# jdfxzzy/DPMN

Measured on AMD Instinct MI355X. Metric: SR images/sec (16x64->32x128, bs=48 per GPU, fp32 forward), higher is better.
Workload: dtype f32; 1 GPU; cfg1: TATT PSN + 3+3 PGRM (embed 96, windows 2/4/8) + CMM, forward-only; per_gpu_batch=48, global_batch=48, ranks=1, batches_in_flight=2, parallelism=dp1 (independent batch shards, no forward collective)

## Files before the change

dpmn_amd/csrc/gemm.hip:

```cpp
#include "gemm_body.h"

namespace {

constexpr int WS_BM = 32, WS_BN = 96;

template <int EPI>
__device__ __forceinline__ void epilogue_fast(f32x4 (&acc)[3][1], int m0, int n0, int ldy, float* y, const float4 (&bias4)[3],
                                              const float* res1, const float* res2, float* red, int bn_cols, int n_block0) {
  const int lane = threadIdx.x & 63;
  const int lm = lane & 15, lq = lane >> 4;
  const size_t off = (size_t)(m0 + lm) * ldy + n0 + lq * 4;
  float4 r1[3], r2[3];
  if (EPI == 3 || EPI == 5) {
#pragma unroll
    for (int nt = 0; nt < 3; ++nt) {
      r1[nt] = *reinterpret_cast<const float4*>(res1 + off + nt * 16);
      if (EPI == 3) r2[nt] = *reinterpret_cast<const float4*>(res2 + off + nt * 16);
    }
  }
#pragma unroll
  for (int nt = 0; nt < 3; ++nt) {
    const float4 b4 = bias4[nt];
    float v[4] = {acc[nt][0][0] + b4.x, acc[nt][0][1] + b4.y, acc[nt][0][2] + b4.z, acc[nt][0][3] + b4.w};
    if (EPI == 2) {
// ... 770 lines not shown
      for (int nt = 0; nt < NT; ++nt) {
        f32x4 c4;
#pragma unroll
        for (int r = 0; r < 4; ++r) {
          float c = cs[nt][r];
          c += xshfl<1>(c); c += xshfl<2>(c); c += xshfl<4>(c); c += xshfl<8>(c);
          c4[r] = c;
        }
        if (lr == 0) *reinterpret_cast<f32x4*>(e.colsum + (size_t)(tile / SUB) * N + n_blk + 16 * nt + 4 * kq) = c4;
      }
    }
  }
}


template <int C, int CG, bool SAVE>
__global__ __launch_bounds__(256, 2) void k_sk_mlp_in(const float* __restrict__ cat, const float* __restrict__ sel, int rows_per_image,
                                                      const float* __restrict__ w_head, const float* __restrict__ b_head,
                                                      const float* __restrict__ feats, const float* __restrict__ shortcut, float* __restrict__ x1,
                                                      const float* __restrict__ ln_w, const float* __restrict__ ln_b, float eps,
                                                      const float* __restrict__ w_fc1, const float* __restrict__ b_fc1, float* __restrict__ y,
                                                      int M, int N, float* __restrict__ v_out, float* __restrict__ n2_out, float p_row,
                                                      unsigned long long seed_row) {
  constexpr int KC = C / 16, KV = C / 4, LDW = C + PAD, BN = 96, NT = 6, G = C / CG, HC = CG / 16, LDH = CG + PAD;
  static_assert(C == 96 && G == 3, "built for dim 96, three window groups");
  extern __shared__ __attribute__((aligned(16))) float smem[];
  float* Ws = smem;
  float* pb = Ws + BN * LDW;
  float* Wh = pb + 3 * BN;
  float* scr = Wh;
  const int tid = threadIdx.x, wave = tid >> 6, lane = tid & 63, lr = lane & 15, kq = lane >> 4;
  const int n_blk = blockIdx.y * BN;
  const int tiles = M / 16;
  const int stride = gridDim.x * 4;
  int tile = blockIdx.x * 4 + wave;
  const bool write_x1 = blockIdx.y == 0;

  constexpr int WL = (BN * KV + 255) / 256;
  float4 wv[WL];
#pragma unroll
  for (int u = 0; u < WL; ++u) {
    const int i = min(tid + u * 256, BN * KV - 1);
    wv[u] = *reinterpret_cast<const float4*>(w_fc1 + (size_t)(n_blk + i / KV) * C + (i % KV) * 4);
  }
  f32x4 xr[G][HC];
  auto load_rows = [&](int t_) {
    const size_t m = (size_t)(t_ < tiles ? t_ : tiles - 1) * 16 + lr;
#pragma unroll
    for (int g = 0; g < G; ++g)
#pragma unroll
      for (int c = 0; c < HC; ++c) xr[g][c] = *reinterpret_cast<const f32x4*>(cat + m * C + g * CG + 16 * c + 4 * kq);
  };
  f32x4 r1[NT], r2[NT];
  auto load_res = [&](int t_) {
    const size_t ro = ((size_t)(t_ < tiles ? t_ : tiles - 1) * 16 + lr) * C + 4 * kq;
#pragma unroll
    for (int nt = 0; nt < NT; ++nt) {
      r1[nt] = *reinterpret_cast<const f32x4*>(feats + ro + 16 * nt);
      r2[nt] = *reinterpret_cast<const f32x4*>(shortcut + ro + 16 * nt);
    }
  };
  load_rows(tile);
  load_res(tile);
#pragma unroll
  for (int u = 0; u < WL; ++u) {
    const int i = tid + u * 256;
    if (i < BN * KV) {
      const int r = i / KV, c4 = (i % KV) * 4;
      float4 v = wv[u];
      if (!SAVE) {
        const float4 gm = *reinterpret_cast<const float4*>(ln_w + c4), bt = *reinterpret_cast<const float4*>(ln_b + c4);
        const float4 wb = make_float4(v.x * bt.x, v.y * bt.y, v.z * bt.z, v.w * bt.w);
        v = make_float4(v.x * gm.x, v.y * gm.y, v.z * gm.z, v.w * gm.w);
        scr[r * KV + c4 / 4] = (wb.x + wb.y) + (wb.z + wb.w);
      }
      *reinterpret_cast<float4*>(Ws + r * LDW + c4) = v;
    }
  }
  __syncthreads();
  if (tid < BN) {
    float bb = b_fc1 ? b_fc1[n_blk + tid] : 0.f, cw = 0.f;
    if (!SAVE)
    for (int k = 0; k < KV; ++k) {
      const float4 v = *reinterpret_cast<const float4*>(Ws + tid * LDW + 4 * k);
      cw += (v.x + v.y) + (v.z + v.w);
      bb += scr[tid * KV + k];
    }
    pb[tid] = bb;
    pb[BN + tid] = cw;
    pb[2 * BN + tid] = b_head ? b_head[tid] : 0.f;
  }
  __syncthreads();
  for (int i = tid; i < C * (CG / 4); i += 256) {
    const int r = i / (CG / 4), c4 = (i % (CG / 4)) * 4;
    *reinterpret_cast<float4*>(Wh + r * LDH + c4) = *reinterpret_cast<const float4*>(w_head + (size_t)r * CG + c4);
  }
  __syncthreads();

  for (; tile < tiles; tile += stride) {
    const size_t m = (size_t)tile * 16 + lr;
    const size_t roff = m * C + 4 * kq;
    f32x4 xb[HC];
    {
      const size_t b = m / rows_per_image;
#pragma unroll
      for (int c = 0; c < HC; ++c) {
        xb[c] = (f32x4){0.f, 0.f, 0.f, 0.f};
#pragma unroll
        for (int g = 0; g < G; ++g) {
          const f32x4 a = *reinterpret_cast<const f32x4*>(sel + (b * G + g) * CG + 16 * c + 4 * kq);
// ... 14 lines not shown
    {
      const float* ha = Wh + lr * LDH + 4 * kq;
#pragma unroll
      for (int c = 0; c < HC; ++c) {
        f32x4 hf[NT];
#pragma unroll
        for (int nt = 0; nt < NT; ++nt) hf[nt] = *reinterpret_cast<const f32x4*>(ha + 16 * nt * LDH + 16 * c);
#pragma unroll
        for (int s4 = 0; s4 < 4; ++s4)
#pragma unroll
          for (int nt = 0; nt < NT; ++nt) x1r[nt] = mfma16(hf[nt][s4], xb[c][s4], x1r[nt]);
      }
    }
#pragma unroll
    for (int nt = 0; nt < NT; ++nt) {
      const f32x4 b4 = *reinterpret_cast<const f32x4*>(pb + 2 * BN + 16 * nt + 4 * kq);
      f32x4 v = x1r[nt] + b4;
      v += r1[nt];
      if (p_row > 0.f) v *= drop_scale(seed_row, (unsigned long long)(m / rows_per_image), p_row, 1.0f / (1.0f - p_row));
      v += r2[nt];
      x1r[nt] = v;
    }
    __builtin_amdgcn_sched_barrier(0);
    load_res(tile + stride);
    __builtin_amdgcn_sched_barrier(0);
    if (write_x1) {
#pragma unroll
      for (int nt = 0; nt < NT; ++nt) *reinterpret_cast<f32x4*>(x1 + roff + 16 * nt) = x1r[nt];
    }
    float mean, rstd;
    {
// ... 10 lines not shown
        q0 = fmaf(d0, d0, q0); q1 = fmaf(d1, d1, q1); q2 = fmaf(d2, d2, q2); q3 = fmaf(d3, d3, q3);
      }
      float q = (q0 + q1) + (q2 + q3);
      q += xshfl<16>(q); q += xshfl<32>(q);
      rstd = 1.0f / sqrtf(q * (1.0f / C) + eps);
    }
    if (SAVE) {
#pragma unroll
      for (int nt = 0; nt < NT; ++nt) {
        const f32x4 gm = *reinterpret_cast<const f32x4*>(ln_w + 16 * nt + 4 * kq), bt = *reinterpret_cast<const f32x4*>(ln_b + 16 * nt + 4 * kq);
#pragma unroll
        for (int r = 0; r < 4; ++r) x1r[nt][r] = (x1r[nt][r] - mean) * rstd * gm[r] + bt[r];
        if (write_x1) *reinterpret_cast<f32x4*>(n2_out + roff + 16 * nt) = x1r[nt];
      }
    }
    f32x4 acc[NT];
#pragma unroll
    for (int nt = 0; nt < NT; ++nt) acc[nt] = (f32x4){0.f, 0.f, 0.f, 0.f};
    const float* wa = Ws + lr * LDW + 4 * kq;
    f32x4 wf[2][NT];
#pragma unroll
    for (int nt = 0; nt < NT; ++nt) wf[0][nt] = *reinterpret_cast<const f32x4*>(wa + 16 * nt * LDW);
#pragma unroll
    for (int c = 0; c < KC; ++c) {
      if (c + 1 < KC) {
#pragma unroll
        for (int nt = 0; nt < NT; ++nt) wf[(c + 1) & 1][nt] = *reinterpret_cast<const f32x4*>(wa + 16 * nt * LDW + 16 * (c + 1));
      }
#pragma unroll
      for (int s4 = 0; s4 < 4; ++s4)
#pragma unroll
        for (int nt = 0; nt < NT; ++nt) acc[nt] = mfma16(wf[c & 1][nt][s4], x1r[c][s4], acc[nt]);
      __builtin_amdgcn_sched_barrier(0);
    }
    const float nm = -mean * rstd;
    const size_t yoff = m * N + n_blk + 4 * kq;
#pragma unroll
    for (int nt = 0; nt < NT; ++nt) {
      const f32x4 b4 = *reinterpret_cast<const f32x4*>(pb + 16 * nt + 4 * kq);
      const f32x4 cw = *reinterpret_cast<const f32x4*>(pb + BN + 16 * nt + 4 * kq);
      f32x4 v;
      if (SAVE) v = acc[nt] + b4;
      else {
#pragma unroll
        for (int r = 0; r < 4; ++r) v[r] = fmaf(acc[nt][r], rstd, fmaf(nm, cw[r], b4[r]));
      }
      *reinterpret_cast<f32x4*>(y + yoff + 16 * nt) = v;
    }
  }
}

template <int K, int PRO, int EPI>
int launch_rowreg(const float* x, int ldx, const float* w, float* y, int ldy, int M, int N, const ProArgs& p, const EpiArgs& e,
                  hipStream_t st) {
  const size_t smem = (size_t)(96 * (K + PAD) + 2 * 96 + (PRO == PRO_LN ? 96 * (K / 4) * 2 : 0)) * sizeof(float);
  static bool attr_set = false;
  if (!attr_set) {
    (void)hipFuncSetAttribute(reinterpret_cast<const void*>(&k_gemm_rowreg<K, PRO, EPI>), hipFuncAttributeMaxDynamicSharedMemorySize, (int)smem);
    attr_set = true;
  }
  const int tiles = M / (EPI == 4 ? 32 : 16), ny = N / 96;
  const bool x3 = (PRO == PRO_NONE || PRO == PRO_LN) && (K == 96 || K == 192) && g_dpmn_x3;
  const int per_cu = x3 ? (K <= 96 ? 2 : 1) : (smem <= 40 * 1024 ? 3 : (smem <= 80 * 1024 ? 2 : 1));
  int gx = 256 * per_cu / ny;
// ... 196 lines not shown
                       dpmn_stream_t stream) {
  return dpmn_sk_mlp_in_drop_f32(cat, attn_vec, w_head, b_head, feats, shortcut, x1, ln_w, ln_b, eps, w_fc1, b_fc1, y, v_out, n2_out, M,
                                 rows_per_image, C, groups, N, 0.f, 0ull, stream);
}

int dpmn_sk_mlp_in_drop_f32(const float* cat, const float* attn_vec, const float* w_head, const float* b_head, const float* feats,
                            const float* shortcut, float* x1, const float* ln_w, const float* ln_b, float eps, const float* w_fc1,
                            const float* b_fc1, float* y, float* v_out, float* n2_out, int M, int rows_per_image, int C, int groups, int N,
                            float p_row, unsigned long long seed_row, dpmn_stream_t stream) {
  DPMN_REQUIRE(p_row >= 0.f && p_row < 1.f, "sk_mlp_in: DropPath rate in [0, 1)");
  DPMN_REQUIRE(cat && attn_vec && w_head && feats && shortcut && x1 && ln_w && ln_b && w_fc1 && y, "sk_mlp_in: null pointer");
  DPMN_REQUIRE((v_out == nullptr) == (n2_out == nullptr), "sk_mlp_in: the two training outputs go together");
  DPMN_REQUIRE(C == 96 && groups == 3 && N % 96 == 0 && M % 16 == 0 && rows_per_image % 16 == 0 && M >= 1024,
               "sk_mlp_in: built for dim 96, three window groups, whole 16-token tiles (dpmn_sk_mlp_in_supported)");
  constexpr int Cc = 96, CG = 32;
  const size_t smem = (size_t)(96 * (Cc + PAD) + 3 * 96 + 96 * (CG + PAD)) * sizeof(float);
  static bool attr_set = false;
  if (!attr_set) {
    (void)hipFuncSetAttribute(reinterpret_cast<const void*>(&k_sk_mlp_in<Cc, CG, false>), hipFuncAttributeMaxDynamicSharedMemorySize, (int)smem);
    (void)hipFuncSetAttribute(reinterpret_cast<const void*>(&k_sk_mlp_in<Cc, CG, true>), hipFuncAttributeMaxDynamicSharedMemorySize, (int)smem);
    attr_set = true;
  }
  const int tiles = M / 16, ny = N / 96;
  int gx = 512 / ny;
  if (gx < 1) gx = 1;
  if (gx * 4 > tiles) gx = cdiv(tiles, 4);
  hipStream_t st = as_stream(stream);
  ProfScope prof(PT_GEMM_WSTAT_LN, st, 2.0 * M * ((double)N * Cc + (double)Cc * CG),
                 4.0 * ((double)M * Cc * 4 + (double)M * N + (double)N * Cc + (double)Cc * CG));
#define SKMLP_LAUNCH(SAVE_) hipLaunchKernelGGL((k_sk_mlp_in<Cc, CG, SAVE_>), dim3(gx, ny), dim3(256), smem, st, cat, attn_vec, rows_per_image, \
                                              w_head, b_head, feats, shortcut, x1, ln_w, ln_b, eps, w_fc1, b_fc1, y, M, N, v_out, n2_out, p_row, seed_row)
  if (g_dpmn_x3)
    dpmn_gemm::x3_launch_sk_mlp_in(cat, attn_vec, rows_per_image, w_head, b_head, feats, shortcut, x1, ln_w, ln_b, eps, w_fc1, b_fc1, y, M, N,
                                   v_out, n2_out, p_row, seed_row, gx, st);
  else if (v_out) SKMLP_LAUNCH(true);
  else SKMLP_LAUNCH(false);
#undef SKMLP_LAUNCH
  DPMN_CHECK_LAUNCH();
  return DPMN_OK;
}

int dpmn_sk_mlp_in_supported(int M, int rows_per_image, int C, int groups, int N) {
  return C == 96 && groups == 3 && N % 96 == 0 && M % 16 == 0 && rows_per_image % 16 == 0 && M >= 1024 && !g_dpmn_bf16;
}

int dpmn_pointwise_wgrad_f32(const float* dz, const float* g, float* dw, int B, int Ch, int L, dpmn_stream_t stream) {
  DPMN_REQUIRE(dz && g && dw && L % 32 == 0 && Ch % 4 == 0, "pointwise_wgrad: bad arguments");
  EpiArgs e{nullptr, nullptr, nullptr, nullptr, ACT_NONE, 0.f, 1};
  dim3 grid(cdiv(Ch, 64), cdiv(Ch, 96), 32);
  if (g_dpmn_x3) dpmn_gemm::x3_launch_kloop(dz, L, g, L, dw, Ch, Ch, Ch, B * L, e, L, (long)Ch * L, (long)Ch * L, grid, as_stream(stream));
  else hipLaunchKernelGGL(k_gemm_kloop, grid, dim3(256), 0, as_stream(stream), dz, L, g, L, dw, Ch, Ch, Ch, B * L, e, L,
                     (long)Ch * L, (long)Ch * L);
// ... 61 lines not shown
```

dpmn_amd/csrc/gemm_body.h:

```cpp
#pragma once
#include <cstdlib>
#include "common.h"

namespace dpmn_gemm {
struct EpiArgs {
  const float* bias;
  const float* res1;
  const float* res2;
  float* colsum;
  int act;
  float slope;
  int atomic;
  long zstride;
  float p_elem = 0.f, p_row = 0.f;
  unsigned long long seed_elem = 0ull, seed_row = 0ull;
  long row_len = 0;
};

struct ProArgs {
  const float* ln_w;
  const float* ln_b;
  float eps;
  const float* sel;
  int rows_per_image;
  int groups;
  const float* addv;
  const float* x2;
  int k1;
};

void x3_launch_kloop(const float* x, int ldx, const float* w, int ldw, float* y, int ldy, int M, int N, int K, const EpiArgs& e, int kb_len,
                     long x_bstride, long w_bstride, dim3 grid, hipStream_t st);
void x3_launch_kloop128(const float* x, const float* w, float* y, int M, int N, int L, int nchunks, int splits, long bstride, long zstride,
                        hipStream_t st);
void x3_launch_pw(const float* g, const float* w, const float* bias, float* z, int B, int Ch, int L, hipStream_t st);
int x3_launch_rowreg(int K, int pro, int epi, const float* x, int ldx, const float* w, float* y, int ldy, int M, int N, const ProArgs& p,
                     const EpiArgs& e, int gx, hipStream_t st);
void x3_launch_sk_mlp_in(const float* cat, const float* sel, int rows_per_image, const float* w_head, const float* b_head, const float* feats,
                         const float* shortcut, float* x1, const float* ln_w, const float* ln_b, float eps, const float* w_fc1, const float* b_fc1,
                         float* y, int M, int N, float* v_out, float* n2_out, float p_row, unsigned long long seed_row, int gx, hipStream_t st);
}

namespace {
using dpmn_gemm::EpiArgs;
using dpmn_gemm::ProArgs;
constexpr int PAD = 4;
enum { PRO_NONE = 0, PRO_LN = 1, PRO_SKSEL = 2, PRO_ADD = 3, PRO_CAT2 = 4 };

template <int NT, int MT, bool FULL = false>
__device__ __forceinline__ void epilogue(f32x4 (&acc)[NT][MT], int m0, int n0, int M, int N, int ldy, float* y,
                                         const EpiArgs& e, float* red , int bn_cols,
                                         int n_block0) {
  const int lane = threadIdx.x & 63;
  const int lm = lane & 15, lq = lane >> 4;
#pragma unroll
// ... 60 lines not shown
```

dpmn_amd/csrc/gemm_rowreg_x3.hip:

```cpp
#include <cstdlib>
#include "gemm_body.h"

namespace {
typedef unsigned u32x4 __attribute__((ext_vector_type(4)));

__device__ __forceinline__ void split_rows8(const f32x4& lo, const f32x4& hi, bf16x8& h, bf16x8& m, bf16x8& l) {
  u32x4 H, M_, L;
  unsigned a, b, c;
  x3_split2t(lo[0], lo[1], a, b, c); H[0] = a; M_[0] = b; L[0] = c;
  x3_split2t(lo[2], lo[3], a, b, c); H[1] = a; M_[1] = b; L[1] = c;
  x3_split2t(hi[0], hi[1], a, b, c); H[2] = a; M_[2] = b; L[2] = c;
  x3_split2t(hi[2], hi[3], a, b, c); H[3] = a; M_[3] = b; L[3] = c;
  h = __builtin_bit_cast(bf16x8, H); m = __builtin_bit_cast(bf16x8, M_); l = __builtin_bit_cast(bf16x8, L);
}

template <int K>
__device__ __forceinline__ void stage_w4(unsigned short* Wb, int r, int c4, const float4& v) {
  constexpr int LDB = K + 8, PL = 96 * LDB;
  uint2 h, m, l;
  x3_split4t(v, h, m, l);
  const int pos = (c4 & ~31) + 8 * ((c4 >> 2) & 3) + 4 * ((c4 >> 4) & 1);
  unsigned short* d = Wb + r * LDB + pos;
  *reinterpret_cast<uint2*>(d) = h;
  *reinterpret_cast<uint2*>(d + PL) = m;
  *reinterpret_cast<uint2*>(d + 2 * PL) = l;
}

template <int K, int NT>
__device__ __forceinline__ void mma_chunk(const unsigned short* Wb, int lr, int kq, int C2, const bf16x8& bh, const bf16x8& bm, const bf16x8& bl,
                                          f32x4 (&acc)[NT]) {
  constexpr int LDB = K + 8, PL = 96 * LDB;
  const unsigned short* wa = Wb + lr * LDB + 32 * C2 + 8 * kq;
  bf16x8 wh[NT], wm[NT], wl[NT];
#pragma unroll
  for (int nt = 0; nt < NT; ++nt) wl[nt] = *reinterpret_cast<const bf16x8*>(wa + 16 * nt * LDB + 2 * PL);
#pragma unroll
  for (int nt = 0; nt < NT; ++nt) wh[nt] = *reinterpret_cast<const bf16x8*>(wa + 16 * nt * LDB);
#pragma unroll
  for (int nt = 0; nt < NT; ++nt) wm[nt] = *reinterpret_cast<const bf16x8*>(wa + 16 * nt * LDB + PL);
#pragma unroll
  for (int nt = 0; nt < NT; ++nt) acc[nt] = mfma16_bf16(wl[nt], bh, acc[nt]);
#pragma unroll
  for (int nt = 0; nt < NT; ++nt) acc[nt] = mfma16_bf16(wh[nt], bl, acc[nt]);
#pragma unroll
  for (int nt = 0; nt < NT; ++nt) acc[nt] = mfma16_bf16(wm[nt], bm, acc[nt]);
#pragma unroll
// ... 132 lines not shown
#pragma unroll
      for (int nt = 0; nt < NT; ++nt) {
        f32x4 c4;
#pragma unroll
        for (int r = 0; r < 4; ++r) {
          float c = cs[nt][r];
          c += xshfl<1>(c); c += xshfl<2>(c); c += xshfl<4>(c); c += xshfl<8>(c);
          c4[r] = c;
        }
        if (lr == 0) *reinterpret_cast<f32x4*>(e.colsum + (size_t)(tile / SUB) * N + n_blk + 16 * nt + 4 * kq) = c4;
      }
    }
  }
}

template <int C, int CG, bool SAVE>
__global__ __launch_bounds__(256, 2) void k_sk_mlp_in_x3(const float* __restrict__ cat, const float* __restrict__ sel, int rows_per_image,
                                                          const float* __restrict__ w_head, const float* __restrict__ b_head,
                                                          const float* __restrict__ feats, const float* __restrict__ shortcut, float* __restrict__ x1,
                                                          const float* __restrict__ ln_w, const float* __restrict__ ln_b, float eps,
                                                          const float* __restrict__ w_fc1, const float* __restrict__ b_fc1, float* __restrict__ y,
                                                          int M, int N, float* __restrict__ v_out, float* __restrict__ n2_out, float p_row,
                                                          unsigned long long seed_row) {
  constexpr int KC = C / 16, K2 = C / 32, KV = C / 4, LDB = C + 8, BN = 96, NT = 6, G = C / CG, HC = CG / 16, LDH = CG + PAD;
  static_assert(C == 96 && G == 3, "built for dim 96, three window groups");
  extern __shared__ __attribute__((aligned(16))) float smem[];
  unsigned short* Wb = reinterpret_cast<unsigned short*>(smem);
  float* pb = smem + 3 * BN * LDB / 2;
  float* Wh = pb + 3 * BN;
  float* scr = Wh;
  const int tid = threadIdx.x, wave = tid >> 6, lane = tid & 63, lr = lane & 15, kq = lane >> 4;
  const int n_blk = blockIdx.y * BN;
  const int tiles = M / 16;
  const int stride = gridDim.x * 4;
  int tile = blockIdx.x * 4 + wave;
  const bool write_x1 = blockIdx.y == 0;

  constexpr int WL = (BN * KV + 255) / 256;
  float4 wv[WL];
#pragma unroll
  for (int u = 0; u < WL; ++u) {
    const int i = min(tid + u * 256, BN * KV - 1);
    wv[u] = *reinterpret_cast<const float4*>(w_fc1 + (size_t)(n_blk + i / KV) * C + (i % KV) * 4);
  }
  f32x4 xr[G][HC];
  auto load_rows = [&](int t_) {
    const size_t m = (size_t)(t_ < tiles ? t_ : tiles - 1) * 16 + lr;
#pragma unroll
    for (int g = 0; g < G; ++g)
#pragma unroll
      for (int c = 0; c < HC; ++c) xr[g][c] = *reinterpret_cast<const f32x4*>(cat + m * C + g * CG + 16 * c + 4 * kq);
  };
  f32x4 r1[NT], r2[NT];
  auto load_res = [&](int t_) {
    const size_t ro = ((size_t)(t_ < tiles ? t_ : tiles - 1) * 16 + lr) * C + 4 * kq;
#pragma unroll
    for (int nt = 0; nt < NT; ++nt) {
      r1[nt] = *reinterpret_cast<const f32x4*>(feats + ro + 16 * nt);
      r2[nt] = *reinterpret_cast<const f32x4*>(shortcut + ro + 16 * nt);
    }
  };
  load_rows(tile);
  load_res(tile);
#pragma unroll
  for (int u = 0; u < WL; ++u) {
    const int i = tid + u * 256;
    if (i < BN * KV) {
      const int r = i / KV, c4 = (i % KV) * 4;
      float4 v = wv[u];
      if (!SAVE) {
        const float4 gm = *reinterpret_cast<const float4*>(ln_w + c4), bt = *reinterpret_cast<const float4*>(ln_b + c4);
        const float4 wb = make_float4(v.x * bt.x, v.y * bt.y, v.z * bt.z, v.w * bt.w);
        v = make_float4(v.x * gm.x, v.y * gm.y, v.z * gm.z, v.w * gm.w);
        scr[(r * KV + c4 / 4) * 2] = (v.x + v.y) + (v.z + v.w);
        scr[(r * KV + c4 / 4) * 2 + 1] = (wb.x + wb.y) + (wb.z + wb.w);
      }
      stage_w4<C>(Wb, r, c4, v);
    }
  }
  __syncthreads();
  if (tid < BN) {
    float bb = b_fc1 ? b_fc1[n_blk + tid] : 0.f, cw = 0.f;
    if (!SAVE)
      for (int k = 0; k < KV; ++k) { cw += scr[(tid * KV + k) * 2]; bb += scr[(tid * KV + k) * 2 + 1]; }
    pb[tid] = bb;
    pb[BN + tid] = cw;
    pb[2 * BN + tid] = b_head ? b_head[tid] : 0.f;
  }
  __syncthreads();
  for (int i = tid; i < C * (CG / 4); i += 256) {
    const int r = i / (CG / 4), c4 = (i % (CG / 4)) * 4;
    *reinterpret_cast<float4*>(Wh + r * LDH + c4) = *reinterpret_cast<const float4*>(w_head + (size_t)r * CG + c4);
  }
  __syncthreads();

  for (; tile < tiles; tile += stride) {
    const size_t m = (size_t)tile * 16 + lr;
    const size_t roff = m * C + 4 * kq;
    f32x4 xb[HC];
    {
      const size_t b = m / rows_per_image;
#pragma unroll
      for (int c = 0; c < HC; ++c) {
        xb[c] = (f32x4){0.f, 0.f, 0.f, 0.f};
#pragma unroll
        for (int g = 0; g < G; ++g) {
          const f32x4 a = *reinterpret_cast<const f32x4*>(sel + (b * G + g) * CG + 16 * c + 4 * kq);
// ... 14 lines not shown
    {
      const float* ha = Wh + lr * LDH + 4 * kq;
#pragma unroll
      for (int c = 0; c < HC; ++c) {
        f32x4 hf[NT];
#pragma unroll
        for (int nt = 0; nt < NT; ++nt) hf[nt] = *reinterpret_cast<const f32x4*>(ha + 16 * nt * LDH + 16 * c);
#pragma unroll
        for (int s4 = 0; s4 < 4; ++s4)
#pragma unroll
          for (int nt = 0; nt < NT; ++nt) x1r[nt] = mfma16(hf[nt][s4], xb[c][s4], x1r[nt]);
      }
    }
#pragma unroll
    for (int nt = 0; nt < NT; ++nt) {
      const f32x4 b4 = *reinterpret_cast<const f32x4*>(pb + 2 * BN + 16 * nt + 4 * kq);
      f32x4 v = x1r[nt] + b4;
      v += r1[nt];
      if (p_row > 0.f) v *= drop_scale(seed_row, (unsigned long long)(m / rows_per_image), p_row, 1.0f / (1.0f - p_row));
      v += r2[nt];
      x1r[nt] = v;
    }
    __builtin_amdgcn_sched_barrier(0);
    load_res(tile + stride);
    __builtin_amdgcn_sched_barrier(0);
    if (write_x1) {
#pragma unroll
      for (int nt = 0; nt < NT; ++nt) *reinterpret_cast<f32x4*>(x1 + roff + 16 * nt) = x1r[nt];
    }
    float mean, rstd;
    {
// ... 10 lines not shown
        q0 = fmaf(d0, d0, q0); q1 = fmaf(d1, d1, q1); q2 = fmaf(d2, d2, q2); q3 = fmaf(d3, d3, q3);
      }
      float q = (q0 + q1) + (q2 + q3);
      q += xshfl<16>(q); q += xshfl<32>(q);
      rstd = 1.0f / sqrtf(q * (1.0f / C) + eps);
    }
    if (SAVE) {
#pragma unroll
      for (int nt = 0; nt < NT; ++nt) {
        const f32x4 gm = *reinterpret_cast<const f32x4*>(ln_w + 16 * nt + 4 * kq), bt = *reinterpret_cast<const f32x4*>(ln_b + 16 * nt + 4 * kq);
#pragma unroll
        for (int r = 0; r < 4; ++r) x1r[nt][r] = (x1r[nt][r] - mean) * rstd * gm[r] + bt[r];
        if (write_x1) *reinterpret_cast<f32x4*>(n2_out + roff + 16 * nt) = x1r[nt];
      }
    }
    f32x4 acc[NT];
#pragma unroll
    for (int nt = 0; nt < NT; ++nt) acc[nt] = (f32x4){0.f, 0.f, 0.f, 0.f};
#pragma unroll
    for (int c2 = 0; c2 < K2; ++c2) {
      bf16x8 bh, bm, bl;
      split_rows8(x1r[2 * c2], x1r[2 * c2 + 1], bh, bm, bl);
      mma_chunk<C, NT>(Wb, lr, kq, c2, bh, bm, bl, acc);
      __builtin_amdgcn_sched_barrier(0);
    }
    const float nm = -mean * rstd;
    const size_t yoff = m * N + n_blk + 4 * kq;
#pragma unroll
    for (int nt = 0; nt < NT; ++nt) {
      const f32x4 b4 = *reinterpret_cast<const f32x4*>(pb + 16 * nt + 4 * kq);
      const f32x4 cw = *reinterpret_cast<const f32x4*>(pb + BN + 16 * nt + 4 * kq);
      f32x4 v;
      if (SAVE) v = acc[nt] + b4;
      else {
#pragma unroll
        for (int r = 0; r < 4; ++r) v[r] = fmaf(acc[nt][r], rstd, fmaf(nm, cw[r], b4[r]));
      }
      *reinterpret_cast<f32x4*>(y + yoff + 16 * nt) = v;
    }
  }
}

template <int K, int PRO, int EPI>
int launch_rr(const float* x, int ldx, const float* w, float* y, int ldy, int M, int N, const ProArgs& p, const EpiArgs& e, int gx, hipStream_t st) {
  const size_t smem = (size_t)3 * 96 * (K + 8) * 2 + (size_t)(2 * 96 + (PRO == PRO_LN ? 96 * (K / 4) * 2 : 0)) * sizeof(float);
  static bool attr_set = false;
  if (!attr_set) {
    (void)hipFuncSetAttribute(reinterpret_cast<const void*>(&k_gemm_rowreg_x3<K, PRO, EPI>), hipFuncAttributeMaxDynamicSharedMemorySize, (int)smem);
    attr_set = true;
  }
  hipLaunchKernelGGL((k_gemm_rowreg_x3<K, PRO, EPI>), dim3(gx, N / 96), dim3(256), smem, st, x, ldx, w, y, ldy, M, N, p, e);
  return 0;
}

template <int K, int PRO>
// ... 12 lines not shown
}
}

namespace dpmn_gemm {
int x3_launch_rowreg(int K, int pro, int epi, const float* x, int ldx, const float* w, float* y, int ldy, int M, int N, const ProArgs& p,
                     const EpiArgs& e, int gx, hipStream_t st) {
  if (K == 96 && pro == PRO_NONE) return launch_rr_epi<96, PRO_NONE>(epi, x, ldx, w, y, ldy, M, N, p, e, gx, st);
  if (K == 96 && pro == PRO_LN) return launch_rr_epi<96, PRO_LN>(epi, x, ldx, w, y, ldy, M, N, p, e, gx, st);
  if (K == 192 && pro == PRO_NONE) return launch_rr_epi<192, PRO_NONE>(epi, x, ldx, w, y, ldy, M, N, p, e, gx, st);
  if (K == 192 && pro == PRO_LN) return launch_rr_epi<192, PRO_LN>(epi, x, ldx, w, y, ldy, M, N, p, e, gx, st);
  return -1;
}

void x3_launch_sk_mlp_in(const float* cat, const float* sel, int rows_per_image, const float* w_head, const float* b_head, const float* feats,
                         const float* shortcut, float* x1, const float* ln_w, const float* ln_b, float eps, const float* w_fc1, const float* b_fc1,
                         float* y, int M, int N, float* v_out, float* n2_out, float p_row, unsigned long long seed_row, int gx, hipStream_t st) {
  constexpr int Cc = 96, CG = 32;
  const size_t smem = (size_t)3 * 96 * (Cc + 8) * 2 + (size_t)(3 * 96 + 96 * (Cc / 4) * 2) * sizeof(float);
  static bool attr_set = false;
  if (!attr_set) {
    (void)hipFuncSetAttribute(reinterpret_cast<const void*>(&k_sk_mlp_in_x3<Cc, CG, false>), hipFuncAttributeMaxDynamicSharedMemorySize, (int)smem);
    (void)hipFuncSetAttribute(reinterpret_cast<const void*>(&k_sk_mlp_in_x3<Cc, CG, true>), hipFuncAttributeMaxDynamicSharedMemorySize, (int)smem);
    attr_set = true;
  }
  if (v_out)
    hipLaunchKernelGGL((k_sk_mlp_in_x3<Cc, CG, true>), dim3(gx, N / 96), dim3(256), smem, st, cat, sel, rows_per_image, w_head, b_head, feats, shortcut,
                       x1, ln_w, ln_b, eps, w_fc1, b_fc1, y, M, N, v_out, n2_out, p_row, seed_row);
  else
    hipLaunchKernelGGL((k_sk_mlp_in_x3<Cc, CG, false>), dim3(gx, N / 96), dim3(256), smem, st, cat, sel, rows_per_image, w_head, b_head, feats, shortcut,
                       x1, ln_w, ln_b, eps, w_fc1, b_fc1, y, M, N, v_out, n2_out, p_row, seed_row);
}
}
```

Measured before the change: 6335 images/s.

## Compute two 96-column fc1 blocks per workgroup in fused SK+MLP-in kernel

The fused selective-kernel head + LN + fc1 kernel now lets each workgroup of 8 waves cover two 96-wide output blocks of fc1 when N/96 is even. The per-tile head GEMM, residual add, LayerNorm statistics and bf16x3 split are then done once per 192 output columns rather than once per 96, so less of that work is repeated across the grid's y dimension. The prologue also drops the shared-memory scratch and one barrier: the LN-folded bias and column sums are computed straight from global weights by each thread. The cost is double the staged weight tile in LDS and 512-thread blocks limited to one per CU, which lowers occupancy, and the grid size is recomputed for the new shape.

```diff
diff --git a/dpmn_amd/csrc/gemm.hip b/dpmn_amd/csrc/gemm.hip
--- a/dpmn_amd/csrc/gemm.hip
+++ b/dpmn_amd/csrc/gemm.hip
@@ -808,33 +808,32 @@
 }
 
 
-template <int C, int CG, bool SAVE>
-__global__ __launch_bounds__(256, 2) void k_sk_mlp_in(const float* __restrict__ cat, const float* __restrict__ sel, int rows_per_image,
-                                                      const float* __restrict__ w_head, const float* __restrict__ b_head,
-                                                      const float* __restrict__ feats, const float* __restrict__ shortcut, float* __restrict__ x1,
-                                                      const float* __restrict__ ln_w, const float* __restrict__ ln_b, float eps,
-                                                      const float* __restrict__ w_fc1, const float* __restrict__ b_fc1, float* __restrict__ y,
-                                                      int M, int N, float* __restrict__ v_out, float* __restrict__ n2_out, float p_row,
-                                                      unsigned long long seed_row) {
+template <int C, int CG, bool SAVE, int NB>
+__global__ __launch_bounds__(NB == 1 ? 256 : 512, NB == 1 ? 2 : 1) void k_sk_mlp_in(
+    const float* __restrict__ cat, const float* __restrict__ sel, int rows_per_image, const float* __restrict__ w_head,
+    const float* __restrict__ b_head, const float* __restrict__ feats, const float* __restrict__ shortcut, float* __restrict__ x1,
+    const float* __restrict__ ln_w, const float* __restrict__ ln_b, float eps, const float* __restrict__ w_fc1,
+    const float* __restrict__ b_fc1, float* __restrict__ y, int M, int N, float* __restrict__ v_out, float* __restrict__ n2_out, float p_row,
+    unsigned long long seed_row) {
+  constexpr int NW = NB == 1 ? 4 : 8, NTH = 64 * NW, ROWS = 96 * NB;
   constexpr int KC = C / 16, KV = C / 4, LDW = C + PAD, BN = 96, NT = 6, G = C / CG, HC = CG / 16, LDH = CG + PAD;
   static_assert(C == 96 && G == 3, "built for dim 96, three window groups");
   extern __shared__ __attribute__((aligned(16))) float smem[];
   float* Ws = smem;
-  float* pb = Ws + BN * LDW;
-  float* Wh = pb + 3 * BN;
-  float* scr = Wh;
+  float* pb = Ws + ROWS * LDW;
+  float* Wh = pb + 2 * ROWS + BN;
   const int tid = threadIdx.x, wave = tid >> 6, lane = tid & 63, lr = lane & 15, kq = lane >> 4;
-  const int n_blk = blockIdx.y * BN;
+  const int n_blk = blockIdx.y * ROWS;
   const int tiles = M / 16;
-  const int stride = gridDim.x * 4;
-  int tile = blockIdx.x * 4 + wave;
+  const int stride = gridDim.x * NW;
+  int tile = blockIdx.x * NW + wave;
   const bool write_x1 = blockIdx.y == 0;
 
-  constexpr int WL = (BN * KV + 255) / 256;
+  constexpr int WL = (ROWS * KV + NTH - 1) / NTH;
   float4 wv[WL];
 #pragma unroll
   for (int u = 0; u < WL; ++u) {
-    const int i = min(tid + u * 256, BN * KV - 1);
+    const int i = min(tid + u * NTH, ROWS * KV - 1);
     wv[u] = *reinterpret_cast<const float4*>(w_fc1 + (size_t)(n_blk + i / KV) * C + (i % KV) * 4);
   }
   f32x4 xr[G][HC];
@@ -858,36 +857,38 @@
   load_res(tile);
 #pragma unroll
   for (int u = 0; u < WL; ++u) {
-    const int i = tid + u * 256;
-    if (i < BN * KV) {
-      const int r = i / KV, c4 = (i % KV) * 4;
+    const int i = tid + u * NTH;
+    if (i < ROWS * KV) {
+      const int r = i / KV, k = i % KV;
       float4 v = wv[u];
       if (!SAVE) {
-        const float4 gm = *reinterpret_cast<const float4*>(ln_w + c4), bt = *reinterpret_cast<const float4*>(ln_b + c4);
-        const float4 wb = make_float4(v.x * bt.x, v.y * bt.y, v.z * bt.z, v.w * bt.w);
+        const float4 gm = *reinterpret_cast<const float4*>(ln_w + 4 * k);
         v = make_float4(v.x * gm.x, v.y * gm.y, v.z * gm.z, v.w * gm.w);
-        scr[r * KV + c4 / 4] = (wb.x + wb.y) + (wb.z + wb.w);
-      }
-      *reinterpret_cast<float4*>(Ws + r * LDW + c4) = v;
-    }
-  }
-  __syncthreads();
-  if (tid < BN) {
+      }
+      *reinterpret_cast<float4*>(Ws + r * LDW + 4 * k) = v;
+    }
+  }
+  for (int i = tid; i < C * (CG / 4); i += NTH) {
+    const int r = i / (CG / 4), k = i % (CG / 4);
+    *reinterpret_cast<float4*>(Wh + r * LDH + 4 * k) = *reinterpret_cast<const float4*>(w_head + (size_t)r * CG + 4 * k);
+  }
+  if (tid < ROWS) {
     float bb = b_fc1 ? b_fc1[n_blk + tid] : 0.f, cw = 0.f;
-    if (!SAVE)
-    for (int k = 0; k < KV; ++k) {
-      const float4 v = *reinterpret_cast<const float4*>(Ws + tid * LDW + 4 * k);
-      cw += (v.x + v.y) + (v.z + v.w);
-      bb += scr[tid * KV + k];
+    if (!SAVE) {
+      const float* wr = w_fc1 + (size_t)(n_blk + tid) * C;
+#pragma unroll 4
+      for (int k = 0; k < KV; ++k) {
+        const float4 w4 = *reinterpret_cast<const float4*>(wr + 4 * k);
+        const float4 gm = *reinterpret_cast<const float4*>(ln_w + 4 * k), bt = *reinterpret_cast<const float4*>(ln_b + 4 * k);
+        const float4 wb = make_float4(w4.x * bt.x, w4.y * bt.y, w4.z * bt.z, w4.w * bt.w);
+        const float4 v = make_float4(w4.x * gm.x, w4.y * gm.y, w4.z * gm.z, w4.w * gm.w);
+        cw += (v.x + v.y) + (v.z + v.w);
+        bb += (wb.x + wb.y) + (wb.z + wb.w);
+      }
     }
     pb[tid] = bb;
-    pb[BN + tid] = cw;
-    pb[2 * BN + tid] = b_head ? b_head[tid] : 0.f;
-  }
-  __syncthreads();
-  for (int i = tid; i < C * (CG / 4); i += 256) {
-    const int r = i / (CG / 4), c4 = (i % (CG / 4)) * 4;
-    *reinterpret_cast<float4*>(Wh + r * LDH + c4) = *reinterpret_cast<const float4*>(w_head + (size_t)r * CG + c4);
+    pb[ROWS + tid] = cw;
+    if (tid < BN) pb[2 * ROWS + tid] = b_head ? b_head[tid] : 0.f;
   }
   __syncthreads();
 
@@ -932,7 +933,7 @@
     }
 #pragma unroll
     for (int nt = 0; nt < NT; ++nt) {
-      const f32x4 b4 = *reinterpret_cast<const f32x4*>(pb + 2 * BN + 16 * nt + 4 * kq);
+      const f32x4 b4 = *reinterpret_cast<const f32x4*>(pb + 2 * ROWS + 16 * nt + 4 * kq);
       f32x4 v = x1r[nt] + b4;
       v += r1[nt];
       if (p_row > 0.f) v *= drop_scale(seed_row, (unsigned long long)(m / rows_per_image), p_row, 1.0f / (1.0f - p_row));
@@ -973,40 +974,67 @@
         if (write_x1) *reinterpret_cast<f32x4*>(n2_out + roff + 16 * nt) = x1r[nt];
       }
     }
-    f32x4 acc[NT];
-#pragma unroll
-    for (int nt = 0; nt < NT; ++nt) acc[nt] = (f32x4){0.f, 0.f, 0.f, 0.f};
-    const float* wa = Ws + lr * LDW + 4 * kq;
-    f32x4 wf[2][NT];
-#pragma unroll
-    for (int nt = 0; nt < NT; ++nt) wf[0][nt] = *reinterpret_cast<const f32x4*>(wa + 16 * nt * LDW);
-#pragma unroll
-    for (int c = 0; c < KC; ++c) {
-      if (c + 1 < KC) {
-#pragma unroll
-        for (int nt = 0; nt < NT; ++nt) wf[(c + 1) & 1][nt] = *reinterpret_cast<const f32x4*>(wa + 16 * nt * LDW + 16 * (c + 1));
-      }
-#pragma unroll
-      for (int s4 = 0; s4 < 4; ++s4)
-#pragma unroll
-        for (int nt = 0; nt < NT; ++nt) acc[nt] = mfma16(wf[c & 1][nt][s4], x1r[c][s4], acc[nt]);
-      __builtin_amdgcn_sched_barrier(0);
-    }
     const float nm = -mean * rstd;
-    const size_t yoff = m * N + n_blk + 4 * kq;
-#pragma unroll
-    for (int nt = 0; nt < NT; ++nt) {
-      const f32x4 b4 = *reinterpret_cast<const f32x4*>(pb + 16 * nt + 4 * kq);
-      const f32x4 cw = *reinterpret_cast<const f32x4*>(pb + BN + 16 * nt + 4 * kq);
-      f32x4 v;
-      if (SAVE) v = acc[nt] + b4;
-      else {
-#pragma unroll
-        for (int r = 0; r < 4; ++r) v[r] = fmaf(acc[nt][r], rstd, fmaf(nm, cw[r], b4[r]));
-      }
-      *reinterpret_cast<f32x4*>(y + yoff + 16 * nt) = v;
-    }
-  }
+#pragma unroll
+    for (int nb = 0; nb < NB; ++nb) {
+      f32x4 acc[NT];
+#pragma unroll
+      for (int nt = 0; nt < NT; ++nt) acc[nt] = (f32x4){0.f, 0.f, 0.f, 0.f};
+      const float* wa = Ws + (nb * BN + lr) * LDW + 4 * kq;
+      f32x4 wf[2][NT];
+#pragma unroll
+      for (int nt = 0; nt < NT; ++nt) wf[0][nt] = *reinterpret_cast<const f32x4*>(wa + 16 * nt * LDW);
+#pragma unroll
+      for (int c = 0; c < KC; ++c) {
+        if (c + 1 < KC) {
+#pragma unroll
+          for (int nt = 0; nt < NT; ++nt) wf[(c + 1) & 1][nt] = *reinterpret_cast<const f32x4*>(wa + 16 * nt * LDW + 16 * (c + 1));
+        }
+#pragma unroll
+        for (int s4 = 0; s4 < 4; ++s4)
+#pragma unroll
+          for (int nt = 0; nt < NT; ++nt) acc[nt] = mfma16(wf[c & 1][nt][s4], x1r[c][s4], acc[nt]);
+        __builtin_amdgcn_sched_barrier(0);
+      }
+      const size_t yoff = m * N + n_blk + nb * BN + 4 * kq;
+#pragma unroll
+      for (int nt = 0; nt < NT; ++nt) {
+        const f32x4 b4 = *reinterpret_cast<const f32x4*>(pb + nb * BN + 16 * nt + 4 * kq);
+        const f32x4 cw = *reinterpret_cast<const f32x4*>(pb + ROWS + nb * BN + 16 * nt + 4 * kq);
+        f32x4 v;
+        if (SAVE) v = acc[nt] + b4;
+        else {
+#pragma unroll
+          for (int r = 0; r < 4; ++r) v[r] = fmaf(acc[nt][r], rstd, fmaf(nm, cw[r], b4[r]));
+        }
+        *reinterpret_cast<f32x4*>(y + yoff + 16 * nt) = v;
+      }
+    }
+  }
+}
+
+template <int NB>
+void launch_sk_mlp_in(const float* cat, const float* sel, int rows_per_image, const float* w_head, const float* b_head, const float* feats,
+                      const float* shortcut, float* x1, const float* ln_w, const float* ln_b, float eps, const float* w_fc1, const float* b_fc1,
+                      float* y, int M, int N, float* v_out, float* n2_out, float p_row, unsigned long long seed_row, hipStream_t st) {
+  constexpr int Cc = 96, CG = 32, NW = NB == 1 ? 4 : 8;
+  constexpr size_t smem = (size_t)(96 * NB * (Cc + PAD) + 2 * 96 * NB + 96 + 96 * (CG + PAD)) * sizeof(float);
+  static bool attr_set = false;
+  if (!attr_set) {
+    (void)hipFuncSetAttribute(reinterpret_cast<const void*>(&k_sk_mlp_in<Cc, CG, false, NB>), hipFuncAttributeMaxDynamicSharedMemorySize, (int)smem);
+    (void)hipFuncSetAttribute(reinterpret_cast<const void*>(&k_sk_mlp_in<Cc, CG, true, NB>), hipFuncAttributeMaxDynamicSharedMemorySize, (int)smem);
+    attr_set = true;
+  }
+  const int tiles = M / 16, ny = N / (96 * NB);
+  int gx = (NB == 1 ? 512 : 256) / ny;
+  if (gx < 1) gx = 1;
+  if (gx * NW > tiles) gx = cdiv(tiles, NW);
+  if (v_out)
+    hipLaunchKernelGGL((k_sk_mlp_in<Cc, CG, true, NB>), dim3(gx, ny), dim3(64 * NW), smem, st, cat, sel, rows_per_image, w_head, b_head, feats,
+                       shortcut, x1, ln_w, ln_b, eps, w_fc1, b_fc1, y, M, N, v_out, n2_out, p_row, seed_row);
+  else
+    hipLaunchKernelGGL((k_sk_mlp_in<Cc, CG, false, NB>), dim3(gx, ny), dim3(64 * NW), smem, st, cat, sel, rows_per_image, w_head, b_head, feats,
+                       shortcut, x1, ln_w, ln_b, eps, w_fc1, b_fc1, y, M, N, v_out, n2_out, p_row, seed_row);
 }
 
 template <int K, int PRO, int EPI>
@@ -1233,28 +1261,19 @@
   DPMN_REQUIRE(C == 96 && groups == 3 && N % 96 == 0 && M % 16 == 0 && rows_per_image % 16 == 0 && M >= 1024,
                "sk_mlp_in: built for dim 96, three window groups, whole 16-token tiles (dpmn_sk_mlp_in_supported)");
   constexpr int Cc = 96, CG = 32;
-  const size_t smem = (size_t)(96 * (Cc + PAD) + 3 * 96 + 96 * (CG + PAD)) * sizeof(float);
-  static bool attr_set = false;
-  if (!attr_set) {
-    (void)hipFuncSetAttribute(reinterpret_cast<const void*>(&k_sk_mlp_in<Cc, CG, false>), hipFuncAttributeMaxDynamicSharedMemorySize, (int)smem);
-    (void)hipFuncSetAttribute(reinterpret_cast<const void*>(&k_sk_mlp_in<Cc, CG, true>), hipFuncAttributeMaxDynamicSharedMemorySize, (int)smem);
-    attr_set = true;
-  }
-  const int tiles = M / 16, ny = N / 96;
-  int gx = 512 / ny;
-  if (gx < 1) gx = 1;
-  if (gx * 4 > tiles) gx = cdiv(tiles, 4);
+  const int ny = N / 96;
   hipStream_t st = as_stream(stream);
   ProfScope prof(PT_GEMM_WSTAT_LN, st, 2.0 * M * ((double)N * Cc + (double)Cc * CG),
                  4.0 * ((double)M * Cc * 4 + (double)M * N + (double)N * Cc + (double)Cc * CG));
-#define SKMLP_LAUNCH(SAVE_) hipLaunchKernelGGL((k_sk_mlp_in<Cc, CG, SAVE_>), dim3(gx, ny), dim3(256), smem, st, cat, attn_vec, rows_per_image, \
-                                              w_head, b_head, feats, shortcut, x1, ln_w, ln_b, eps, w_fc1, b_fc1, y, M, N, v_out, n2_out, p_row, seed_row)
   if (g_dpmn_x3)
     dpmn_gemm::x3_launch_sk_mlp_in(cat, attn_vec, rows_per_image, w_head, b_head, feats, shortcut, x1, ln_w, ln_b, eps, w_fc1, b_fc1, y, M, N,
-                                   v_out, n2_out, p_row, seed_row, gx, st);
-  else if (v_out) SKMLP_LAUNCH(true);
-  else SKMLP_LAUNCH(false);
-#undef SKMLP_LAUNCH
+                                   v_out, n2_out, p_row, seed_row, st);
+  else if (ny % 2 == 0)
+    launch_sk_mlp_in<2>(cat, attn_vec, rows_per_image, w_head, b_head, feats, shortcut, x1, ln_w, ln_b, eps, w_fc1, b_fc1, y, M, N, v_out, n2_out,
+                        p_row, seed_row, st);
+  else
+    launch_sk_mlp_in<1>(cat, attn_vec, rows_per_image, w_head, b_head, feats, shortcut, x1, ln_w, ln_b, eps, w_fc1, b_fc1, y, M, N, v_out, n2_out,
+                        p_row, seed_row, st);
   DPMN_CHECK_LAUNCH();
   return DPMN_OK;
 }
diff --git a/dpmn_amd/csrc/gemm_body.h b/dpmn_amd/csrc/gemm_body.h
--- a/dpmn_amd/csrc/gemm_body.h
+++ b/dpmn_amd/csrc/gemm_body.h
@@ -38,7 +38,7 @@
                      const EpiArgs& e, int gx, hipStream_t st);
 void x3_launch_sk_mlp_in(const float* cat, const float* sel, int rows_per_image, const float* w_head, const float* b_head, const float* feats,
                          const float* shortcut, float* x1, const float* ln_w, const float* ln_b, float eps, const float* w_fc1, const float* b_fc1,
-                         float* y, int M, int N, float* v_out, float* n2_out, float p_row, unsigned long long seed_row, int gx, hipStream_t st);
+                         float* y, int M, int N, float* v_out, float* n2_out, float p_row, unsigned long long seed_row, hipStream_t st);
 }
 
 namespace {
diff --git a/dpmn_amd/csrc/gemm_rowreg_x3.hip b/dpmn_amd/csrc/gemm_rowreg_x3.hip
--- a/dpmn_amd/csrc/gemm_rowreg_x3.hip
+++ b/dpmn_amd/csrc/gemm_rowreg_x3.hip
@@ -14,9 +14,9 @@
   h = __builtin_bit_cast(bf16x8, H); m = __builtin_bit_cast(bf16x8, M_); l = __builtin_bit_cast(bf16x8, L);
 }
 
-template <int K>
+template <int K, int R = 96>
 __device__ __forceinline__ void stage_w4(unsigned short* Wb, int r, int c4, const float4& v) {
-  constexpr int LDB = K + 8, PL = 96 * LDB;
+  constexpr int LDB = K + 8, PL = R * LDB;
   uint2 h, m, l;
   x3_split4t(v, h, m, l);
   const int pos = (c4 & ~31) + 8 * ((c4 >> 2) & 3) + 4 * ((c4 >> 4) & 1);
@@ -26,10 +26,10 @@
   *reinterpret_cast<uint2*>(d + 2 * PL) = l;
 }
 
-template <int K, int NT>
+template <int K, int NT, int R = 96>
 __device__ __forceinline__ void mma_chunk(const unsigned short* Wb, int lr, int kq, int C2, const bf16x8& bh, const bf16x8& bm, const bf16x8& bl,
                                           f32x4 (&acc)[NT]) {
-  constexpr int LDB = K + 8, PL = 96 * LDB;
+  constexpr int LDB = K + 8, PL = R * LDB;
   const unsigned short* wa = Wb + lr * LDB + 32 * C2 + 8 * kq;
   bf16x8 wh[NT], wm[NT], wl[NT];
 #pragma unroll
@@ -192,33 +192,33 @@
   }
 }
 
-template <int C, int CG, bool SAVE>
-__global__ __launch_bounds__(256, 2) void k_sk_mlp_in_x3(const float* __restrict__ cat, const float* __restrict__ sel, int rows_per_image,
+template <int C, int CG, bool SAVE, int NB>
+__global__ __launch_bounds__(NB == 1 ? 256 : 512, NB == 1 ? 2 : 1) void k_sk_mlp_in_x3(const float* __restrict__ cat, const float* __restrict__ sel, int rows_per_image,
                                                           const float* __restrict__ w_head, const float* __restrict__ b_head,
                                                           const float* __restrict__ feats, const float* __restrict__ shortcut, float* __restrict__ x1,
                                                           const float* __restrict__ ln_w, const float* __restrict__ ln_b, float eps,
                                                           const float* __restrict__ w_fc1, const float* __restrict__ b_fc1, float* __restrict__ y,
                                                           int M, int N, float* __restrict__ v_out, float* __restrict__ n2_out, float p_row,
                                                           unsigned long long seed_row) {
+  constexpr int NW = NB == 1 ? 4 : 8, NTH = 64 * NW, ROWS = 96 * NB;
   constexpr int KC = C / 16, K2 = C / 32, KV = C / 4, LDB = C + 8, BN = 96, NT = 6, G = C / CG, HC = CG / 16, LDH = CG + PAD;
   static_assert(C == 96 && G == 3, "built for dim 96, three window groups");
   extern __shared__ __attribute__((aligned(16))) float smem[];
   unsigned short* Wb = reinterpret_cast<unsigned short*>(smem);
-  float* pb = smem + 3 * BN * LDB / 2;
-  float* Wh = pb + 3 * BN;
-  float* scr = Wh;
+  float* pb = smem + 3 * ROWS * LDB / 2;
+  float* Wh = pb + 2 * ROWS + BN;
   const int tid = threadIdx.x, wave = tid >> 6, lane = tid & 63, lr = lane & 15, kq = lane >> 4;
-  const int n_blk = blockIdx.y * BN;
+  const int n_blk = blockIdx.y * ROWS;
   const int tiles = M / 16;
-  const int stride = gridDim.x * 4;
-  int tile = blockIdx.x * 4 + wave;
+  const int stride = gridDim.x * NW;
+  int tile = blockIdx.x * NW + wave;
   const bool write_x1 = blockIdx.y == 0;
 
-  constexpr int WL = (BN * KV + 255) / 256;
+  constexpr int WL = (ROWS * KV + NTH - 1) / NTH;
   float4 wv[WL];
 #pragma unroll
   for (int u = 0; u < WL; ++u) {
-    const int i = min(tid + u * 256, BN * KV - 1);
+    const int i = min(tid + u * NTH, ROWS * KV - 1);
     wv[u] = *reinterpret_cast<const float4*>(w_fc1 + (size_t)(n_blk + i / KV) * C + (i % KV) * 4);
   }
   f32x4 xr[G][HC];
@@ -242,33 +242,38 @@
   load_res(tile);
 #pragma unroll
   for (int u = 0; u < WL; ++u) {
-    const int i = tid + u * 256;
-    if (i < BN * KV) {
+    const int i = tid + u * NTH;
+    if (i < ROWS * KV) {
       const int r = i / KV, c4 = (i % KV) * 4;
       float4 v = wv[u];
       if (!SAVE) {
-        const float4 gm = *reinterpret_cast<const float4*>(ln_w + c4), bt = *reinterpret_cast<const float4*>(ln_b + c4);
-        const float4 wb = make_float4(v.x * bt.x, v.y * bt.y, v.z * bt.z, v.w * bt.w);
+        const float4 gm = *reinterpret_cast<const float4*>(ln_w + c4);
         v = make_float4(v.x * gm.x, v.y * gm.y, v.z * gm.z, v.w * gm.w);
-        scr[(r * KV + c4 / 4) * 2] = (v.x + v.y) + (v.z + v.w);
-        scr[(r * KV + c4 / 4) * 2 + 1] = (wb.x + wb.y) + (wb.z + wb.w);
-      }
-      stage_w4<C>(Wb, r, c4, v);
-    }
-  }
-  __syncthreads();
-  if (tid < BN) {
-    float bb = b_fc1 ? b_fc1[n_blk + tid] : 0.f, cw = 0.f;
-    if (!SAVE)
-      for (int k = 0; k < KV; ++k) { cw += scr[(tid * KV + k) * 2]; bb += scr[(tid * KV + k) * 2 + 1]; }
-    pb[tid] = bb;
-    pb[BN + tid] = cw;
-    pb[2 * BN + tid] = b_head ? b_head[tid] : 0.f;
-  }
-  __syncthreads();
-  for (int i = tid; i < C * (CG / 4); i += 256) {
+      }
+      stage_w4<C, ROWS>(Wb, r, c4, v);
+    }
+  }
+  for (int i = tid; i < C * (CG / 4); i += NTH) {
     const int r = i / (CG / 4), c4 = (i % (CG / 4)) * 4;
     *reinterpret_cast<float4*>(Wh + r * LDH + c4) = *reinterpret_cast<const float4*>(w_head + (size_t)r * CG + c4);
+  }
+  if (tid < ROWS) {
+    float bb = b_fc1 ? b_fc1[n_blk + tid] : 0.f, cw = 0.f;
+    if (!SAVE) {
+      const float* wr = w_fc1 + (size_t)(n_blk + tid) * C;
+#pragma unroll 4
+      for (int k = 0; k < KV; ++k) {
+        const float4 w4 = *reinterpret_cast<const float4*>(wr + 4 * k);
+        const float4 gm = *reinterpret_cast<const float4*>(ln_w + 4 * k), bt = *reinterpret_cast<const float4*>(ln_b + 4 * k);
+        const float4 wb = make_float4(w4.x * bt.x, w4.y * bt.y, w4.z * bt.z, w4.w * bt.w);
+        const float4 v = make_float4(w4.x * gm.x, w4.y * gm.y, w4.z * gm.z, w4.w * gm.w);
+        cw += (v.x + v.y) + (v.z + v.w);
+        bb += (wb.x + wb.y) + (wb.z + wb.w);
+      }
+    }
+    pb[tid] = bb;
+    pb[ROWS + tid] = cw;
+    if (tid < BN) pb[2 * ROWS + tid] = b_head ? b_head[tid] : 0.f;
   }
   __syncthreads();
 
@@ -313,7 +318,7 @@
     }
 #pragma unroll
     for (int nt = 0; nt < NT; ++nt) {
-      const f32x4 b4 = *reinterpret_cast<const f32x4*>(pb + 2 * BN + 16 * nt + 4 * kq);
+      const f32x4 b4 = *reinterpret_cast<const f32x4*>(pb + 2 * ROWS + 16 * nt + 4 * kq);
       f32x4 v = x1r[nt] + b4;
       v += r1[nt];
       if (p_row > 0.f) v *= drop_scale(seed_row, (unsigned long long)(m / rows_per_image), p_row, 1.0f / (1.0f - p_row));
@@ -354,31 +359,59 @@
         if (write_x1) *reinterpret_cast<f32x4*>(n2_out + roff + 16 * nt) = x1r[nt];
       }
     }
-    f32x4 acc[NT];
-#pragma unroll
-    for (int nt = 0; nt < NT; ++nt) acc[nt] = (f32x4){0.f, 0.f, 0.f, 0.f};
-#pragma unroll
-    for (int c2 = 0; c2 < K2; ++c2) {
-      bf16x8 bh, bm, bl;
-      split_rows8(x1r[2 * c2], x1r[2 * c2 + 1], bh, bm, bl);
-      mma_chunk<C, NT>(Wb, lr, kq, c2, bh, bm, bl, acc);
-      __builtin_amdgcn_sched_barrier(0);
-    }
+    bf16x8 bh[K2], bm[K2], bl[K2];
+#pragma unroll
+    for (int c2 = 0; c2 < K2; ++c2) split_rows8(x1r[2 * c2], x1r[2 * c2 + 1], bh[c2], bm[c2], bl[c2]);
     const float nm = -mean * rstd;
-    const size_t yoff = m * N + n_blk + 4 * kq;
-#pragma unroll
-    for (int nt = 0; nt < NT; ++nt) {
-      const f32x4 b4 = *reinterpret_cast<const f32x4*>(pb + 16 * nt + 4 * kq);
-      const f32x4 cw = *reinterpret_cast<const f32x4*>(pb + BN + 16 * nt + 4 * kq);
-      f32x4 v;
-      if (SAVE) v = acc[nt] + b4;
-      else {
-#pragma unroll
-        for (int r = 0; r < 4; ++r) v[r] = fmaf(acc[nt][r], rstd, fmaf(nm, cw[r], b4[r]));
-      }
-      *reinterpret_cast<f32x4*>(y + yoff + 16 * nt) = v;
-    }
-  }
+#pragma unroll
+    for (int nb = 0; nb < NB; ++nb) {
+      f32x4 acc[NT];
+#pragma unroll
+      for (int nt = 0; nt < NT; ++nt) acc[nt] = (f32x4){0.f, 0.f, 0.f, 0.f};
+#pragma unroll
+      for (int c2 = 0; c2 < K2; ++c2) {
+        mma_chunk<C, NT, ROWS>(Wb + nb * BN * LDB, lr, kq, c2, bh[c2], bm[c2], bl[c2], acc);
+        __builtin_amdgcn_sched_barrier(0);
+      }
+      const size_t yoff = m * N + n_blk + nb * BN + 4 * kq;
+#pragma unroll
+      for (int nt = 0; nt < NT; ++nt) {
+        const f32x4 b4 = *reinterpret_cast<const f32x4*>(pb + nb * BN + 16 * nt + 4 * kq);
+        const f32x4 cw = *reinterpret_cast<const f32x4*>(pb + ROWS + nb * BN + 16 * nt + 4 * kq);
+        f32x4 v;
+        if (SAVE) v = acc[nt] + b4;
+        else {
+#pragma unroll
+          for (int r = 0; r < 4; ++r) v[r] = fmaf(acc[nt][r], rstd, fmaf(nm, cw[r], b4[r]));
+        }
+        *reinterpret_cast<f32x4*>(y + yoff + 16 * nt) = v;
+      }
+    }
+  }
+}
+
+template <int NB>
+void launch_skm(const float* cat, const float* sel, int rows_per_image, const float* w_head, const float* b_head, const float* feats,
+                const float* shortcut, float* x1, const float* ln_w, const float* ln_b, float eps, const float* w_fc1, const float* b_fc1, float* y,
+                int M, int N, float* v_out, float* n2_out, float p_row, unsigned long long seed_row, hipStream_t st) {
+  constexpr int Cc = 96, CG = 32, NW = NB == 1 ? 4 : 8;
+  constexpr size_t smem = (size_t)3 * 96 * NB * (Cc + 8) * 2 + (size_t)(2 * 96 * NB + 96 + 96 * (CG + PAD)) * sizeof(float);
+  static bool attr_set = false;
+  if (!attr_set) {
+    (void)hipFuncSetAttribute(reinterpret_cast<const void*>(&k_sk_mlp_in_x3<Cc, CG, false, NB>), hipFuncAttributeMaxDynamicSharedMemorySize, (int)smem);
+    (void)hipFuncSetAttribute(reinterpret_cast<const void*>(&k_sk_mlp_in_x3<Cc, CG, true, NB>), hipFuncAttributeMaxDynamicSharedMemorySize, (int)smem);
+    attr_set = true;
+  }
+  const int tiles = M / 16, ny = N / (96 * NB);
+  int gx = (NB == 1 ? 512 : 256) / ny;
+  if (gx < 1) gx = 1;
+  if (gx * NW > tiles) gx = (tiles + NW - 1) / NW;
+  if (v_out)
+    hipLaunchKernelGGL((k_sk_mlp_in_x3<Cc, CG, true, NB>), dim3(gx, ny), dim3(64 * NW), smem, st, cat, sel, rows_per_image, w_head, b_head, feats,
+                       shortcut, x1, ln_w, ln_b, eps, w_fc1, b_fc1, y, M, N, v_out, n2_out, p_row, seed_row);
+  else
+    hipLaunchKernelGGL((k_sk_mlp_in_x3<Cc, CG, false, NB>), dim3(gx, ny), dim3(64 * NW), smem, st, cat, sel, rows_per_image, w_head, b_head, feats,
+                       shortcut, x1, ln_w, ln_b, eps, w_fc1, b_fc1, y, M, N, v_out, n2_out, p_row, seed_row);
 }
 
 template <int K, int PRO, int EPI>
@@ -421,20 +454,10 @@
 
 void x3_launch_sk_mlp_in(const float* cat, const float* sel, int rows_per_image, const float* w_head, const float* b_head, const float* feats,
                          const float* shortcut, float* x1, const float* ln_w, const float* ln_b, float eps, const float* w_fc1, const float* b_fc1,
-                         float* y, int M, int N, float* v_out, float* n2_out, float p_row, unsigned long long seed_row, int gx, hipStream_t st) {
-  constexpr int Cc = 96, CG = 32;
-  const size_t smem = (size_t)3 * 96 * (Cc + 8) * 2 + (size_t)(3 * 96 + 96 * (Cc / 4) * 2) * sizeof(float);
-  static bool attr_set = false;
-  if (!attr_set) {
-    (void)hipFuncSetAttribute(reinterpret_cast<const void*>(&k_sk_mlp_in_x3<Cc, CG, false>), hipFuncAttributeMaxDynamicSharedMemorySize, (int)smem);
-    (void)hipFuncSetAttribute(reinterpret_cast<const void*>(&k_sk_mlp_in_x3<Cc, CG, true>), hipFuncAttributeMaxDynamicSharedMemorySize, (int)smem);
-    attr_set = true;
-  }
-  if (v_out)
-    hipLaunchKernelGGL((k_sk_mlp_in_x3<Cc, CG, true>), dim3(gx, N / 96), dim3(256), smem, st, cat, sel, rows_per_image, w_head, b_head, feats, shortcut,
-                       x1, ln_w, ln_b, eps, w_fc1, b_fc1, y, M, N, v_out, n2_out, p_row, seed_row);
+                         float* y, int M, int N, float* v_out, float* n2_out, float p_row, unsigned long long seed_row, hipStream_t st) {
+  if ((N / 96) % 2 == 0)
+    launch_skm<2>(cat, sel, rows_per_image, w_head, b_head, feats, shortcut, x1, ln_w, ln_b, eps, w_fc1, b_fc1, y, M, N, v_out, n2_out, p_row, seed_row, st);
   else
-    hipLaunchKernelGGL((k_sk_mlp_in_x3<Cc, CG, false>), dim3(gx, N / 96), dim3(256), smem, st, cat, sel, rows_per_image, w_head, b_head, feats, shortcut,
-                       x1, ln_w, ln_b, eps, w_fc1, b_fc1, y, M, N, v_out, n2_out, p_row, seed_row);
-}
-}
+    launch_skm<1>(cat, sel, rows_per_image, w_head, b_head, feats, shortcut, x1, ln_w, ln_b, eps, w_fc1, b_fc1, y, M, N, v_out, n2_out, p_row, seed_row, st);
+}
+}
```

New measurement: 6387 images/s, median of 6. About the same (+0.8%).
